# supranational/sppark

Hardware: NVIDIA H100
Metric: BLS12-381 G1 MSM/s @2^26 points (higher is better)
Workload: dtype u32x12 (384-bit Montgomery integers)

## Files before the change

### include/sppark_b200.h

```cpp
#ifndef SPPARK_B200_H
#define SPPARK_B200_H

#include <stddef.h>
#include <stdint.h>

#ifdef __cplusplus
extern "C" {
#endif

typedef struct RustError {
    int   code;
    char *message;
#ifdef __cplusplus
    typedef struct RustError by_value;
#endif
} RustError;


enum { SPPARK_NTT_NN = 0, SPPARK_NTT_NR = 1, SPPARK_NTT_RN = 2, SPPARK_NTT_RR = 3,
       SPPARK_NTT_BB = 4 };
enum { SPPARK_NTT_FORWARD = 0, SPPARK_NTT_INVERSE = 1 };
enum { SPPARK_NTT_STANDARD = 0, SPPARK_NTT_COSET = 1 };


// ... 44 lines not shown
                                     uint32_t lg_blowup, void *stream);

RustError sppark_b200_ntt_batch_dev(int field, void *d_inout, uint32_t lg_domain_size, size_t batch,
                                    int ntt_order, int ntt_direction, int ntt_type, void *stream);
RustError sppark_b200_lde_batch_dev(int field, void *d_out, void *d_in, uint32_t lg_domain_size,
                                    uint32_t lg_blowup, size_t batch, void *stream);
RustError sppark_b200_ntt_batch(int field, size_t device_id, void *inout, uint32_t lg_domain_size,
                                size_t batch, int ntt_order, int ntt_direction, int ntt_type);

RustError sppark_b200_prefix_op_dev(int field, int op, void *d_out, const void *d_inp, size_t len, void *stream);
RustError sppark_b200_div_by_x_minus_z_dev(int field, void *d_inout, size_t len, const void *z, int rotate,
                                           void *stream);
RustError sppark_b200_evaluate_dev(int field, void *d_ret, const void *d_x, size_t n, const void *d_coeffs,
                                   size_t len, void *stream);
RustError sppark_b200_batch_inverse_dev(int field, void *d_out, const void *d_inp, size_t len, void *stream);

RustError sppark_b200_ntt_slab_pass(int field, int which, const void *d_in, void *d_out,
                                    uint32_t lg_domain_size, uint32_t lg_g, uint32_t rank,
                                    int ntt_direction, void *stream);

RustError sppark_b200_ntt_slab_pass_p2p(int field, const void *d_in, void *const *peer_recv,
                                        uint32_t lg_domain_size, uint32_t lg_g, uint32_t rank,
                                        int ntt_direction, void *stream);
RustError sppark_b200_ntt_sharded(int field, void *inout, uint32_t lg_domain_size, int ntt_direction,
                                  const int *device_ids, size_t ndev);

RustError sppark_b200_peer_alloc(size_t bytes, void **d_ptr, void *ipc_handle_64);
RustError sppark_b200_peer_open(const void *ipc_handle_64, void **d_ptr);
RustError sppark_b200_peer_close(void *d_ptr);
RustError sppark_b200_peer_free(void *d_ptr);

RustError sppark_b200_msm(int curve, void *out_jacobian, const void *points_affine,
                          size_t npoints, const void *scalars, size_t ffi_affine_sz);
RustError sppark_b200_msm_ex(int curve, void *out_jacobian, const void *points_affine,
                             size_t npoints, const void *scalars, size_t ffi_affine_sz,
                             int scalars_mont);
RustError sppark_b200_msm_sharded(int curve, void *out_jacobian, const void *points_affine, size_t npoints,
                                  const void *scalars, size_t ffi_affine_sz, int scalars_mont,
                                  const int *device_ids, size_t ndev);
typedef struct sppark_b200_msm_ctx sppark_b200_msm_ctx;
RustError sppark_b200_msm_ctx_create(int curve, const void *points_affine, size_t npoints,
                                     size_t ffi_affine_sz, sppark_b200_msm_ctx **out);
RustError sppark_b200_msm_ctx_invoke(sppark_b200_msm_ctx *ctx, void *out_jacobian, const void *scalars,
                                     size_t npoints, int scalars_mont);
void      sppark_b200_msm_ctx_free(sppark_b200_msm_ctx *ctx);
RustError sppark_b200_msm_dev(int curve, void *out_jacobian, const void *d_points,
                              size_t npoints, const void *d_scalars, void *stream);

RustError sppark_b200_generate_points_dev(int curve, void *d_out, size_t n, void *stream);
RustError sppark_b200_msm_combine(int curve, void *out_jacobian, const void *partials, size_t count);

RustError sppark_b200_selftest_field(int field, int op, size_t n, void *r, const void *a, const void *b);
RustError sppark_b200_selftest_word_field(int field, int op, size_t n, void *r, const void *a, const void *b);

size_t      sppark_b200_ngpus(void);
int         sppark_b200_sm_count(int device_id);
const char *sppark_b200_version(void);
uint64_t    sppark_b200_launch_count(void);
void        sppark_b200_profile_enable(int on);
int         sppark_b200_profile_read(const char **names, float *ms, int cap);

#ifdef __cplusplus
}
#endif
#endif
```

### sppark_b200/_lib.py

```python
import ctypes as C
import os

HERE = os.path.dirname(os.path.abspath(__file__))
LIB_PATH = os.environ.get("SPPARK_B200_LIB") or os.path.join(HERE, "libsppark_b200.so")


class RustError(C.Structure):
    _fields_ = [("code", C.c_int), ("message", C.c_void_p)]


class GpuPtr(C.Structure):
    _fields_ = [("inner", C.c_void_p)]


class SpparkError(RuntimeError):
    def __init__(self, code, message):
        super().__init__(f"sppark_b200 error {code}: {message}")
        self.code = code


_lib = None

_SIGS = {
    "mult_pippenger": [C.c_void_p, C.c_void_p, C.c_size_t, C.c_void_p],
    "mult_pippenger_inf": [C.c_void_p, C.c_void_p, C.c_size_t, C.c_void_p, C.c_size_t],
    "mult_pippenger_fp2_inf": [C.c_void_p, C.c_void_p, C.c_size_t, C.c_void_p, C.c_size_t],
    "compute_ntt": [C.c_size_t, C.c_void_p, C.c_uint32, C.c_int, C.c_int, C.c_int],
    "sppark_b200_ntt": [C.c_int, C.c_size_t, C.c_void_p, C.c_uint32, C.c_int, C.c_int, C.c_int],
    "sppark_b200_ntt_dev": [C.c_int, C.c_void_p, C.c_uint32, C.c_int, C.c_int, C.c_int, C.c_void_p],
    "sppark_b200_lde": [C.c_int, C.c_size_t, C.c_void_p, C.c_uint32, C.c_uint32, C.c_void_p],
    "sppark_b200_ntt_slab_pass": [C.c_int, C.c_int, C.c_void_p, C.c_void_p, C.c_uint32, C.c_uint32, C.c_uint32,
                                  C.c_int, C.c_void_p],
    "sppark_b200_ntt_slab_pass_p2p": [C.c_int, C.c_void_p, C.c_void_p, C.c_uint32, C.c_uint32, C.c_uint32,
                                      C.c_int, C.c_void_p],
    "sppark_b200_peer_alloc": [C.c_size_t, C.POINTER(C.c_void_p), C.c_void_p],
    "sppark_b200_peer_open": [C.c_void_p, C.POINTER(C.c_void_p)],
    "sppark_b200_peer_close": [C.c_void_p],
    "sppark_b200_peer_free": [C.c_void_p],
    "sppark_b200_msm": [C.c_int, C.c_void_p, C.c_void_p, C.c_size_t, C.c_void_p, C.c_size_t],
    "sppark_b200_msm_ex": [C.c_int, C.c_void_p, C.c_void_p, C.c_size_t, C.c_void_p, C.c_size_t, C.c_int],
    "sppark_b200_msm_ctx_create": [C.c_int, C.c_void_p, C.c_size_t, C.c_size_t, C.POINTER(C.c_void_p)],
    "sppark_b200_msm_ctx_invoke": [C.c_void_p, C.c_void_p, C.c_void_p, C.c_size_t, C.c_int],
    "sppark_b200_msm_dev": [C.c_int, C.c_void_p, C.c_void_p, C.c_size_t, C.c_void_p, C.c_void_p],
    "sppark_b200_generate_points_dev": [C.c_int, C.c_void_p, C.c_size_t, C.c_void_p],
    "sppark_b200_msm_combine": [C.c_int, C.c_void_p, C.c_void_p, C.c_size_t],
    "sppark_b200_selftest_field": [C.c_int, C.c_int, C.c_size_t, C.c_void_p, C.c_void_p, C.c_void_p],
    "sppark_b200_lde_powers_dev": [C.c_int, C.c_void_p, C.c_uint32, C.c_void_p],
    "sppark_b200_lde_expand_dev": [C.c_int, C.c_void_p, C.c_void_p, C.c_uint32, C.c_uint32, C.c_void_p],
    "sppark_b200_ntt_batch_dev": [C.c_int, C.c_void_p, C.c_uint32, C.c_size_t, C.c_int, C.c_int, C.c_int, C.c_void_p],
    "sppark_b200_lde_batch_dev": [C.c_int, C.c_void_p, C.c_void_p, C.c_uint32, C.c_uint32, C.c_size_t, C.c_void_p],
    "sppark_b200_ntt_batch": [C.c_int, C.c_size_t, C.c_void_p, C.c_uint32, C.c_size_t, C.c_int, C.c_int, C.c_int],
    "sppark_b200_msm_sharded": [C.c_int, C.c_void_p, C.c_void_p, C.c_size_t, C.c_void_p, C.c_size_t, C.c_int, C.c_void_p, C.c_size_t],
    "sppark_b200_ntt_sharded": [C.c_int, C.c_void_p, C.c_uint32, C.c_int, C.c_void_p, C.c_size_t],
    "sppark_b200_selftest_word_field": [C.c_int, C.c_int, C.c_size_t, C.c_void_p, C.c_void_p, C.c_void_p],
    "sppark_b200_prefix_op_dev": [C.c_int, C.c_int, C.c_void_p, C.c_void_p, C.c_size_t, C.c_void_p],
    "sppark_b200_div_by_x_minus_z_dev": [C.c_int, C.c_void_p, C.c_size_t, C.c_void_p, C.c_int, C.c_void_p],
    "sppark_b200_evaluate_dev": [C.c_int, C.c_void_p, C.c_void_p, C.c_size_t, C.c_void_p, C.c_size_t, C.c_void_p],
    "sppark_b200_batch_inverse_dev": [C.c_int, C.c_void_p, C.c_void_p, C.c_size_t, C.c_void_p],
}

EXPORTS = list(_SIGS) + ["cuda_available", "drop_error_message", "sppark_b200_sm_count", "sppark_b200_ngpus",
                         "sppark_b200_version", "sppark_b200_launch_count",
                         "sppark_b200_profile_enable", "sppark_b200_profile_read",
                         "drop_gpu_ptr_t", "clone_gpu_ptr_t", "sppark_b200_msm_ctx_free", "sppark_b200_gpu_ptr_alloc",
                         "sppark_b200_gpu_ptr_get", "sppark_b200_gpu_ptr_refs"]


def lib():
    global _lib
    if _lib is None:
        if not os.path.exists(LIB_PATH):
            raise ImportError(f"{LIB_PATH} not built: run `python -m sppark_b200.build` "
                              "(there is no CPU fallback)")
        l = C.CDLL(LIB_PATH)
        for name, args in _SIGS.items():
            fn = getattr(l, name)
            fn.argtypes = args
            fn.restype = RustError
        l.cuda_available.restype = C.c_int
        l.drop_error_message.argtypes = [C.c_void_p]
        l.sppark_b200_sm_count.argtypes = [C.c_int]
        l.sppark_b200_version.restype = C.c_char_p
        l.sppark_b200_launch_count.restype = C.c_uint64
        l.sppark_b200_msm_ctx_free.argtypes = [C.c_void_p]
        l.sppark_b200_msm_ctx_free.restype = None
        l.drop_gpu_ptr_t.argtypes = [C.POINTER(GpuPtr)]
        l.clone_gpu_ptr_t.argtypes = [C.POINTER(GpuPtr)]
        l.clone_gpu_ptr_t.restype = GpuPtr
        l.sppark_b200_gpu_ptr_alloc.argtypes = [C.c_size_t]
        l.sppark_b200_gpu_ptr_alloc.restype = GpuPtr
        l.sppark_b200_gpu_ptr_get.argtypes = [C.POINTER(GpuPtr)]
        l.sppark_b200_gpu_ptr_get.restype = C.c_void_p
        l.sppark_b200_gpu_ptr_refs.argtypes = [C.POINTER(GpuPtr)]
        l.sppark_b200_gpu_ptr_refs.restype = C.c_size_t
        l.sppark_b200_profile_enable.argtypes = [C.c_int]
        l.sppark_b200_profile_read.argtypes = [C.POINTER(C.c_char_p), C.POINTER(C.c_float), C.c_int]
        l.sppark_b200_profile_read.restype = C.c_int
        _lib = l
    return _lib


def check(err):
    if err.code != 0:
        msg = C.cast(err.message, C.c_char_p).value.decode() if err.message else ""
        if err.message:
            lib().drop_error_message(err.message)
        raise SpparkError(err.code, msg)
# ... 16 lines not shown
```

### sppark_b200/csrc/msm/msm.cuh

```cuda
#pragma once
#include "../util/gpu.cuh"
#include "msm_core.cuh"
#include "msm_pair.cuh"

namespace msm {

#ifndef SPPARK_B200_ACC_THREADS
# define SPPARK_B200_ACC_THREADS 128
#endif
#ifndef SPPARK_B200_ACC_MIN_BLOCKS
# define SPPARK_B200_ACC_MIN_BLOCKS 3
#endif
constexpr uint32_t ACC_THREADS = SPPARK_B200_ACC_THREADS;
constexpr uint32_t HEAVY_THREADS = 128;

static __global__ void count_kernel(const Config cfg, const uint32_t* scalars, uint32_t* counts)
{
    for (uint32_t i = blockIdx.x * blockDim.x + threadIdx.x; i < cfg.npoints; i += gridDim.x * blockDim.x)
        count_body(cfg, scalars, counts, i);
}


static __global__ void __launch_bounds__(1024)
scan_kernel(const Config cfg, const uint32_t* counts, uint32_t* offsets, uint32_t* cursor,
            uint32_t* ctrl, uint32_t* heavy_list, uint32_t* chunk_map)
{
    __shared__ uint32_t warp_tot[32];
    const uint32_t w = blockIdx.x, nb = 1u << cfg.lg_nb;
    const uint32_t lane = threadIdx.x & 31, wid = threadIdx.x >> 5;
    const size_t base = (size_t)w << cfg.lg_nb;
    uint32_t carry = 0;
    for (uint32_t t0 = 0; t0 < nb; t0 += 4096) {
        const uint32_t b = t0 + threadIdx.x * 4;
        uint4 c = make_uint4(0, 0, 0, 0);
        if (b < nb) c = *reinterpret_cast<const uint4*>(counts + base + b);
        const uint32_t s = c.x + c.y + c.z + c.w;
        uint32_t x = s;
#pragma unroll
        for (uint32_t d = 1; d < 32; d <<= 1) {
            uint32_t y = __shfl_up_sync(0xffffffffu, x, d);
            if (lane >= d) x += y;
        }
        if (lane == 31) warp_tot[wid] = x;
        __syncthreads();
        if (wid == 0) {
            uint32_t t = warp_tot[lane];
#pragma unroll
            for (uint32_t d = 1; d < 32; d <<= 1) {
                uint32_t y = __shfl_up_sync(0xffffffffu, t, d);
                if (lane >= d) t += y;
            }
            warp_tot[lane] = t;
        }
        __syncthreads();
        uint4 r;
        r.x = carry + (wid ? warp_tot[wid - 1] : 0) + x - s;
        r.y = r.x + c.x;
        r.z = r.y + c.y;
        r.w = r.z + c.z;
        carry += warp_tot[31];
        if (b < nb) {
            *reinterpret_cast<uint4*>(offsets + base + b) = r;
            *reinterpret_cast<uint4*>(cursor + base + b) = r;
            const uint32_t cc[4] = {c.x, c.y, c.z, c.w};
#pragma unroll
            for (uint32_t k = 0; k < 4; k++) {
                if (cc[k] > cfg.heavy) {
                    uint32_t h = atomicAdd(&ctrl[1], 1), nch = (cc[k] + cfg.heavy_chunk - 1) / cfg.heavy_chunk;
                    uint32_t first_chunk = atomicAdd(&ctrl[2], nch);
                    heavy_list[3 * h] = (uint32_t)(base + b + k);
                    heavy_list[3 * h + 1] = first_chunk;
                    heavy_list[3 * h + 2] = nch;
                    for (uint32_t q = 0; q < nch; q++) chunk_map[first_chunk + q] = h;
                }
            }
        }
        __syncthreads();
    }
}

static __global__ void scatter_kernel(const Config cfg, const uint32_t* scalars, uint32_t* cursor, uint32_t* sorted,
                                      uint32_t w0, uint32_t w1)
{
    for (uint32_t i = blockIdx.x * blockDim.x + threadIdx.x; i < cfg.npoints; i += gridDim.x * blockDim.x)
        scatter_body(cfg, scalars, cursor, sorted, i, w0, w1);
}

static __global__ void pair_counts_kernel(const Config cfg, const uint32_t* counts, uint32_t* counts1, uint32_t nslots)
{
    for (uint32_t t = blockIdx.x * blockDim.x + threadIdx.x; t < nslots; t += gridDim.x * blockDim.x)
        pair_counts_body(cfg, counts, counts1, t);
}

static __global__ void __launch_bounds__(1024)
pair_scan_kernel(const Config cfg, const uint32_t* counts1, uint32_t* off1, uint32_t* wintotal)
{
    __shared__ uint32_t warp_tot[32];
    const uint32_t w = blockIdx.x, nb = 1u << cfg.lg_nb, lane = threadIdx.x & 31, wid = threadIdx.x >> 5;
    const size_t base = (size_t)w << cfg.lg_nb;
    uint32_t carry = 0;
    for (uint32_t t0 = 0; t0 < nb; t0 += 4096) {
        const uint32_t b = t0 + threadIdx.x * 4;
        uint4 c = make_uint4(0, 0, 0, 0);
        if (b < nb) c = *reinterpret_cast<const uint4*>(counts1 + base + b);
        const uint32_t s = c.x + c.y + c.z + c.w;
        uint32_t x = s;
#pragma unroll
        for (uint32_t d = 1; d < 32; d <<= 1) {
            uint32_t y = __shfl_up_sync(0xffffffffu, x, d);
            if (lane >= d) x += y;
        }
        if (lane == 31) warp_tot[wid] = x;
        __syncthreads();
        if (wid == 0) {
            uint32_t t = warp_tot[lane];
#pragma unroll
            for (uint32_t d = 1; d < 32; d <<= 1) {
                uint32_t y = __shfl_up_sync(0xffffffffu, t, d);
                if (lane >= d) t += y;
            }
            warp_tot[lane] = t;
        }
        __syncthreads();
        uint4 r;
        r.x = carry + (wid ? warp_tot[wid - 1] : 0) + x - s;
        r.y = r.x + c.x;
        r.z = r.y + c.y;
        r.w = r.z + c.z;
        carry += warp_tot[31];
        if (b < nb) *reinterpret_cast<uint4*>(off1 + base + b) = r;
        __syncthreads();
    }
    if (threadIdx.x == 0) wintotal[w] = carry;
}

static __global__ void pair_winbase_kernel(const Config cfg, const uint32_t* wintotal, uint32_t* winbase)
{
    if (blockIdx.x || threadIdx.x) return;
// ... 260 lines not shown
    }
}

template<class F>
__global__ void __launch_bounds__(32)
finish_par_kernel(const Config cfg, const uint32_t* winR, uint32_t* out_jacobian)
{
    __shared__ F slots[Par4<F>::NS];
    if (threadIdx.x >= 4) return;
    Par4<F> p(slots, slots + 4, threadIdx.x);
    {
        const ec::xyzz_t<F> top = load_bucket<F>(winR, cfg.nwins - 1);
        if (p.lane == 0) { slots[Par4<F>::sX] = top.X; slots[Par4<F>::sY] = top.Y; slots[Par4<F>::sZZZ] = top.ZZZ; slots[Par4<F>::sZZ] = top.ZZ; }
        p.sync();
    }
    for (uint32_t w = cfg.nwins - 1; w-- > 0;) {
        for (uint32_t d = 0; d < cfg.wbits; d++) p.dbl();
        p.add(load_bucket<F>(winR, w));
    }
    const bool inf = p.is_inf();
    const F ZZ = slots[Par4<F>::sZZ];
    const F Yf = slots[Par4<F>::sY], ZZZf = slots[Par4<F>::sZZZ];
    const F r = F::mul_shared(p.pick(slots[Par4<F>::sX], Yf, Yf, Yf), p.pick(ZZ, ZZZf, ZZZf, ZZZf));
    if (p.lane < 2)
        for (int k = 0; k < F::N; k++) out_jacobian[p.lane * F::N + k] = inf ? 0 : r.l[k];
    if (p.lane == 2)
        for (int k = 0; k < F::N; k++) out_jacobian[2 * F::N + k] = inf ? 0 : ZZ.l[k];
}

static __global__ void pack_points_kernel(const uint8_t* in, size_t stride, uint32_t words, bool has_flag,
                                   uint32_t* out, uint32_t npoints)
{
    for (uint32_t i = blockIdx.x * blockDim.x + threadIdx.x; i < npoints; i += gridDim.x * blockDim.x) {
        const uint32_t* src = reinterpret_cast<const uint32_t*>(in + (size_t)i * stride);
        bool inf = has_flag && (in[(size_t)i * stride + 4 * words] & 1);
        for (uint32_t k = 0; k < words; k++) out[(size_t)i * words + k] = inf ? 0 : src[k];
    }
}

template<class F>
class msm_t {
    const gpu_t& gpu;
    static constexpr uint32_t PW = 2 * F::N, BW = 4 * F::N, JW = 3 * F::N;

public:
    explicit msm_t(const gpu_t& g) : gpu(g) {}

    struct Job {
        Config cfg;
        size_t nslots, slice_cap;
        uint32_t lg_l, items1;
        uint8_t* blob;
        uint32_t *counts, *offsets, *cursor, *ctrl, *heavy_list, *chunk_map, *partials, *sorted, *buckets;
        uint32_t *R[2], *S[2];
        uint32_t slices_done;
        bool pair;
        size_t pair_bound;
        uint32_t pair_threads;
        uint32_t *counts1, *off1, *wintotal, *winbase, *sums, *pre, *totals;
        cudaStream_t owner;
        Job() : blob(nullptr), owner(nullptr) {}
        Job(const Job&) = delete;
        Job& operator=(const Job&) = delete;
        Job(Job&& o) noexcept { memcpy((void*)this, (const void*)&o, sizeof(Job)); o.blob = nullptr; }
        ~Job() { if (blob) (void)cudaFreeAsync(blob, owner); }
    };

    Job begin(size_t total_points, size_t slice_cap, cudaStream_t stream)
    {
        if (total_points >= (1ull << 31))
            throw cuda_error(-(int)cudaErrorInvalidValue, "msm: npoints must be < 2^31");
        Job j;
        j.cfg = make_config(total_points);
        j.cfg.npoints = (uint32_t)slice_cap;
        j.slice_cap = slice_cap;
        j.nslots = (size_t)j.cfg.nwins << j.cfg.lg_nb;
        j.lg_l = j.cfg.lg_nb > 12 ? j.cfg.lg_nb - 12 : 0;
        j.items1 = j.cfg.nwins << (j.cfg.lg_nb - j.lg_l);
        j.slices_done = 0;
        const size_t entries = (size_t)j.cfg.nwins * slice_cap;
        const size_t heavy_cap = entries / (j.cfg.heavy + 1) + 1;
        const size_t chunk_cap = entries / j.cfg.heavy_chunk + heavy_cap;
        size_t off = 0;
        auto take = [&](size_t bytes) { size_t o = off; off += (bytes + 255) & ~(size_t)255; return o; };
        const size_t o_counts = take(j.nslots * 4), o_offsets = take(j.nslots * 4), o_cursor = take(j.nslots * 4);
        const size_t o_ctrl = take(16), o_heavy = take(heavy_cap * 12), o_cmap = take(chunk_cap * 4);
        const size_t o_partials = take(chunk_cap * BW * 4);
        const size_t o_sorted = take(entries * 4);
        const size_t o_buckets = take(j.nslots * BW * 4);
        const size_t o_r0 = take((size_t)j.items1 * BW * 4), o_s0 = take((size_t)j.items1 * BW * 4);
        const size_t o_r1 = take((size_t)j.items1 * BW * 4 / 2 + 4096), o_s1 = take((size_t)j.items1 * BW * 4 / 2 + 4096);
        const char* pair_env = getenv("SPPARK_B200_MSM_PAIR");
        j.pair = pair_env && atoi(pair_env) != 0 && entries + j.nslots < (1ull << 31);
        j.pair_bound = (entries + std::min<size_t>(entries, j.nslots) + 1) / 2;
        j.pair_threads = (uint32_t)std::min<size_t>((j.pair_bound + PAIR_K - 1) / PAIR_K, (size_t)1 << 21);
        size_t o_c1 = 0, o_o1 = 0, o_wt = 0, o_wb = 0, o_sums = 0, o_pre = 0, o_tot = 0;
        if (j.pair) {
            o_c1 = take(j.nslots * 4); o_o1 = take(j.nslots * 4);
            o_wt = take((j.cfg.nwins + 1) * 4); o_wb = take((j.cfg.nwins + 1) * 4);
            o_sums = take(j.pair_bound * 2 * F::N * 4);
            o_pre = take((size_t)j.pair_threads * PAIR_K * F::N * 4);
            o_tot = take((size_t)j.pair_threads * F::N * 4);
        }
        CUDA_OK(cudaMallocAsync((void**)&j.blob, off, stream));
        j.owner = stream;
        auto U32 = [&](size_t o) { return reinterpret_cast<uint32_t*>(j.blob + o); };
        j.counts = U32(o_counts); j.offsets = U32(o_offsets); j.cursor = U32(o_cursor);
        j.ctrl = U32(o_ctrl); j.heavy_list = U32(o_heavy); j.chunk_map = U32(o_cmap);
        j.partials = U32(o_partials); j.sorted = U32(o_sorted); j.buckets = U32(o_buckets);
        j.R[0] = U32(o_r0); j.S[0] = U32(o_s0); j.R[1] = U32(o_r1); j.S[1] = U32(o_s1);
        j.counts1 = U32(o_c1); j.off1 = U32(o_o1); j.wintotal = U32(o_wt); j.winbase = U32(o_wb);
        j.sums = U32(o_sums); j.pre = U32(o_pre); j.totals = U32(o_tot);
        g_profile.reset();
        return j;
    }

    void slice(Job& j, const uint32_t* d_points, const uint32_t* d_scalars, size_t n, cudaStream_t stream)
    {
        if (n == 0) return;
        Config cfg = j.cfg;
        cfg.npoints = (uint32_t)n;
        cfg.merge = j.slices_done ? 1 : 0;
        const uint32_t sms = (uint32_t)gpu.sm_count();
        g_profile.mark("sort", stream);
        CUDA_OK(cudaMemsetAsync(j.counts, 0, j.nslots * 4, stream));
        CUDA_OK(cudaMemsetAsync(j.ctrl, 0, 16, stream));
        const uint32_t nblk = (uint32_t)std::min<size_t>((n + 255) / 256, (size_t)sms * 16);
        count_kernel<<<nblk, 256, 0, stream>>>(cfg, d_scalars, j.counts);
        COUNT_LAUNCH();
        scan_kernel<<<cfg.nwins, 1024, 0, stream>>>(cfg, j.counts, j.offsets, j.cursor, j.ctrl, j.heavy_list, j.chunk_map);
        COUNT_LAUNCH();
        bool per_window = n >= (1u << 18);
        if (const char* env = getenv("SPPARK_B200_MSM_SCATTER")) per_window = atoi(env) != 0;
        if (per_window) {
            for (uint32_t w = 0; w < cfg.nwins; w++) {
                scatter_kernel<<<nblk, 256, 0, stream>>>(cfg, d_scalars, j.cursor, j.sorted, w, w + 1);
                COUNT_LAUNCH();
            }
        } else {
            scatter_kernel<<<nblk, 256, 0, stream>>>(cfg, d_scalars, j.cursor, j.sorted, 0, cfg.nwins);
            COUNT_LAUNCH();
        }
        CUDA_OK(cudaGetLastError());

        g_profile.mark("accumulate", stream);
        int occ = 1;
        CUDA_OK(cudaOccupancyMaxActiveBlocksPerMultiprocessor(&occ, accumulate_kernel<F>, ACC_THREADS, 0));
        if (occ < 1) occ = 1;
        size_t want = (j.nslots + ACC_THREADS - 1) / ACC_THREADS;
        uint32_t acc_blocks = (uint32_t)std::min<size_t>(want, (size_t)sms * occ);
        if (j.pair) {
            const uint32_t nslots = (uint32_t)j.nslots;
            pair_counts_kernel<<<sms * 8, 256, 0, stream>>>(cfg, j.counts, j.counts1, nslots);
            pair_scan_kernel<<<cfg.nwins, 1024, 0, stream>>>(cfg, j.counts1, j.off1, j.wintotal);
            pair_winbase_kernel<<<1, 32, 0, stream>>>(cfg, j.wintotal, j.winbase);
            const size_t bound = ((size_t)cfg.nwins * n + std::min<size_t>((size_t)cfg.nwins * n, j.nslots) + 1) / 2;
            const size_t per_launch = (size_t)j.pair_threads * PAIR_K;
            for (size_t o0 = 0; o0 < bound; o0 += per_launch) {
                const uint32_t nth = (uint32_t)std::min<size_t>(j.pair_threads, (bound - o0 + PAIR_K - 1) / PAIR_K);
                pair_forward_kernel<F><<<(nth + 127) / 128, 128, 0, stream>>>(
                    cfg, d_points, j.sorted, j.offsets, j.counts, j.counts1, j.off1, j.winbase, (uint32_t)o0, nth, j.pre, j.totals);
                pair_invert_kernel<F><<<((nth + PAIR_M - 1) / PAIR_M + 127) / 128, 128, 0, stream>>>(j.totals, nth);
                pair_backward_kernel<F><<<(nth + 127) / 128, 128, 0, stream>>>(
                    cfg, d_points, j.sorted, j.offsets, j.counts, j.counts1, j.off1, j.winbase, (uint32_t)o0, nth, j.pre, j.totals, j.sums);
                COUNT_LAUNCH(); COUNT_LAUNCH(); COUNT_LAUNCH();
            }
            CUDA_OK(cudaGetLastError());
            g_profile.mark("accumulate_sums", stream);
            accumulate_direct_kernel<F><<<acc_blocks, ACC_THREADS, 0, stream>>>(cfg, j.sums, j.offsets, j.counts, j.buckets,
                                                                               j.ctrl, j.counts1, j.off1, j.winbase);
        } else {
            accumulate_kernel<F><<<acc_blocks, ACC_THREADS, 0, stream>>>(cfg, d_points, j.sorted, j.offsets, j.counts,
                                                                        j.buckets, j.ctrl);
        }
        COUNT_LAUNCH();
        g_profile.mark("heavy", stream);
        heavy_chunks_kernel<F><<<sms * 4, HEAVY_THREADS, HEAVY_THREADS * BW * 4, stream>>>(
            cfg, d_points, j.sorted, j.offsets, j.counts, j.ctrl, j.heavy_list, j.chunk_map, j.partials);
        COUNT_LAUNCH();
        heavy_fold_kernel<F><<<sms, HEAVY_THREADS, HEAVY_THREADS * BW * 4, stream>>>(cfg, j.ctrl, j.heavy_list,
                                                                                    j.partials, j.buckets);
        COUNT_LAUNCH();
        CUDA_OK(cudaGetLastError());
        if (getenv("SPPARK_B200_MSM_DEBUG")) {
            uint32_t dbg[3];
            CUDA_OK(cudaMemcpyAsync(dbg, j.ctrl, 12, cudaMemcpyDeviceToHost, stream));
            CUDA_OK(cudaStreamSynchronize(stream));
            fprintf(stderr, "[msm] slice %u n=%u wbits=%u nwins=%u heavy_thr=%u tasks_claimed=%u nheavy=%u nchunks=%u acc_blocks=%u\n",
                    j.slices_done, cfg.npoints, cfg.wbits, cfg.nwins, cfg.heavy, dbg[0], dbg[1], dbg[2], acc_blocks);
        }
        j.slices_done++;
    }

    void finish(Job& j, uint32_t* d_out, cudaStream_t stream)
    {
        if (j.slices_done == 0) {
// ... 44 lines not shown
```

### sppark_b200/csrc/msm/msm_bls12_381.cu

```cuda
#include "msm_host.cuh"

RustError msm_host_bls12_381(void* out, const void* points, size_t npoints, const void* scalars,
                             size_t stride, bool has_flag, bool mont)
{
    return msm_host<ff::bls12_381_fp_t>(out, points, npoints, scalars, stride, has_flag,
                                        mont ? scalars_from_mont<ff::bls12_381_fr_t> : nullptr);
}
RustError msm_dev_bls12_381(void* out, const void* d_points, size_t npoints, const void* d_scalars, void* stream)
{   return msm_dev<ff::bls12_381_fp_t>(out, d_points, npoints, d_scalars, stream);   }

RustError gen_points_bls12_381(void* d_out, size_t n, void* stream)
{   return gen_points_dev<ff::bls12_381_g1_gen>(d_out, n, stream);   }
RustError combine_bls12_381(void* out, const void* partials, size_t count)
{   return combine_host<ff::bls12_381_fp_t>(out, partials, count);   }

extern "C" RustError mult_pippenger(void* out, const void* points, size_t npoints, const void* scalars)
{   return msm_host_bls12_381(out, points, npoints, scalars, 96, false, false);   }

extern "C" RustError mult_pippenger_inf(void* out, const void* points, size_t npoints,
                                        const void* scalars, size_t ffi_affine_sz)
{   return msm_host_bls12_381(out, points, npoints, scalars, ffi_affine_sz, true, false);   }

template<class F>
__global__ void selftest_kernel(int op, size_t n, uint32_t* r, const uint32_t* a, const uint32_t* b)
// ... 7 lines not shown
    case 1: z = x + y; break;
    case 2: z = x - y; break;
    case 3: z = x.sqr(); break;
    case 4: z = F::mul_shared(x, y); break;
    case 5: z = F::sqr_shared(x); break;
    default: z = F::msub_shared(x, y, y, x.sqr()); break;
    }
    for (int k = 0; k < F::N; k++) r[i * F::N + k] = z.l[k];
}

template<class F>
static RustError selftest(int op, size_t n, void* r, const void* a, const void* b)
{
    try {
        const gpu_t& gpu = select_gpu(-1);
        const stream_t& s = gpu[0];
        size_t bytes = n * F::N * 4;
        dev_ptr_t<uint32_t> da(n * F::N, s), db(n * F::N, s), dr(n * F::N, s);
        s.HtoD(da, a, bytes);
        s.HtoD(db, b, bytes);
        selftest_kernel<F><<<(unsigned)((n + 127) / 128), 128, 0, s>>>(op, n, dr, da, db);
        COUNT_LAUNCH();
        CUDA_OK(cudaGetLastError());
        s.DtoH(r, dr, bytes);
        s.sync();
    } catch (const cuda_error& e) {
        return rust_err(e.code(), e.what());
    }
    return rust_ok();
}

extern "C" RustError sppark_b200_selftest_field(int field, int op, size_t n, void* r, const void* a, const void* b)
{
    switch (field) {
    case 0: return selftest<ff::bls12_381_fp_t>(op, n, r, a, b);
    case 1: return selftest<ff::bls12_381_fr_t>(op, n, r, a, b);
    case 2: return selftest<ff::pallas_fp_t>(op, n, r, a, b);
    case 3: return selftest<ff::vesta_fp_t>(op, n, r, a, b);
    case 4: return selftest<ff::bn254_fp_t>(op, n, r, a, b);
    case 5: return selftest<ff::bn254_fr_t>(op, n, r, a, b);
    case 6: return selftest<ff::bls12_377_fp_t>(op, n, r, a, b);
    case 7: return selftest<ff::bls12_377_fr_t>(op, n, r, a, b);
    default: return rust_err(-(int)cudaErrorInvalidValue, "selftest: unknown field");
    }
}

RustError msm_preload_bls12_381(const void* points, size_t npoints, size_t stride, bool has_flag, void** d_points)
{   return msm_preload<ff::bls12_381_fp_t>(points, npoints, stride, has_flag, d_points);   }
RustError msm_resident_bls12_381(void* out, const void* d_points, size_t npoints, const void* scalars, bool mont)
{
    return msm_host<ff::bls12_381_fp_t>(out, nullptr, npoints, scalars, 0, false, mont ? scalars_from_mont<ff::bls12_381_fr_t> : nullptr,
                      (const uint32_t*)d_points);
}
```

### sppark_b200/csrc/msm/msm_core.cuh

```cuda
#pragma once
#include <algorithm>
#include "../ec/xyzz.cuh"

namespace msm {

struct Config {
    uint32_t wbits;
    uint32_t nwins;
    uint32_t lg_nb;
    uint32_t npoints;
    uint32_t heavy;
    uint32_t heavy_chunk;
    uint32_t merge;
};

HD uint32_t atomic_inc(uint32_t* p, uint32_t v = 1)
{
#if defined(__CUDA_ARCH__)
    return atomicAdd(p, v);
#else
    uint32_t old = *p;
    *p += v;
    return old;
#endif
// ... 4 lines not shown
    uint32_t carry;
    HD explicit Digits(const uint32_t* p) : carry(0)
    {
#if defined(__CUDA_ARCH__)
        uint4 a = reinterpret_cast<const uint4*>(p)[0], b = reinterpret_cast<const uint4*>(p)[1];
        s[0] = a.x; s[1] = a.y; s[2] = a.z; s[3] = a.w;
        s[4] = b.x; s[5] = b.y; s[6] = b.z; s[7] = b.w;
#else
        for (int i = 0; i < 8; i++) s[i] = p[i];
#endif
        s[7] &= 0x7fffffffu;
    }
    HD bool next(uint32_t w, uint32_t c, uint32_t& bucket, uint32_t& neg)
    {
        uint32_t off = w * c, i = off >> 5, sh = off & 31;
        uint32_t lo = i < 8 ? s[i] : 0, hi = i + 1 < 8 ? s[i + 1] : 0;
        uint32_t raw = sh ? (lo >> sh) | (hi << (32 - sh)) : lo;
        raw = (c < 32 ? raw & ((1u << c) - 1) : raw) + carry;
        const uint32_t half = 1u << (c - 1);
        if (raw > half) {
            neg = 1;
            carry = 1;
            raw = (1u << c) - raw;
        } else {
            neg = 0;
            carry = 0;
        }
        bucket = raw - 1;
        return raw != 0;
    }
};

HD void count_body(const Config& cfg, const uint32_t* scalars, uint32_t* counts, uint32_t i)
{
    Digits d(scalars + 8 * (size_t)i);
    for (uint32_t w = 0; w < cfg.nwins; w++) {
        uint32_t b, neg;
        if (d.next(w, cfg.wbits, b, neg))
            atomic_inc(&counts[((size_t)w << cfg.lg_nb) + b]);
    }
}

HD void scatter_body(const Config& cfg, const uint32_t* scalars, uint32_t* cursor,
                     uint32_t* sorted, uint32_t i, uint32_t w0, uint32_t w1)
{
    Digits d(scalars + 8 * (size_t)i);
    for (uint32_t w = 0; w < w1; w++) {
        uint32_t b, neg;
        if (d.next(w, cfg.wbits, b, neg) && w >= w0) {
            uint32_t pos = atomic_inc(&cursor[((size_t)w << cfg.lg_nb) + b]);
            sorted[(size_t)w * cfg.npoints + pos] = i | (neg << 31);
        }
    }
}

template<class F>
HD ec::affine_t<F> load_point(const uint32_t* points, uint32_t entry)
{
    constexpr int W = 2 * F::N;
    const uint32_t* p = points + (size_t)(entry & 0x7fffffffu) * W;
    ec::affine_t<F> a;
#if defined(__CUDA_ARCH__)
    static_assert(W % 4 == 0, "affine point must be a whole number of 16-byte words");
    uint32_t buf[W];
#pragma unroll
    for (int k = 0; k < W / 4; k++) {
        uint4 v = __ldg(reinterpret_cast<const uint4*>(p) + k);
        buf[4 * k] = v.x; buf[4 * k + 1] = v.y; buf[4 * k + 2] = v.z; buf[4 * k + 3] = v.w;
    }
#pragma unroll
    for (int k = 0; k < F::N; k++) { a.X.l[k] = buf[k]; a.Y.l[k] = buf[F::N + k]; }
#else
    for (int k = 0; k < F::N; k++) { a.X.l[k] = p[k]; a.Y.l[k] = p[F::N + k]; }
#endif
    if (entry >> 31) a.Y = a.Y.neg();
    return a;
}

template<class F>
HD void store_bucket(uint32_t* buckets, size_t slot, const ec::xyzz_t<F>& b)
{
    constexpr int W = 4 * F::N;
    uint32_t* p = buckets + slot * W;
#pragma unroll
    for (int k = 0; k < F::N; k++) {
        p[k] = b.X.l[k]; p[F::N + k] = b.Y.l[k]; p[2 * F::N + k] = b.ZZZ.l[k]; p[3 * F::N + k] = b.ZZ.l[k];
    }
}

template<class F>
HD ec::xyzz_t<F> load_bucket(const uint32_t* buckets, size_t slot)
{
    constexpr int W = 4 * F::N;
    const uint32_t* p = buckets + slot * W;
    ec::xyzz_t<F> b;
#pragma unroll
    for (int k = 0; k < F::N; k++) {
        b.X.l[k] = p[k]; b.Y.l[k] = p[F::N + k]; b.ZZZ.l[k] = p[2 * F::N + k]; b.ZZ.l[k] = p[3 * F::N + k];
    }
    return b;
}

template<class F, bool DIRECT = false>
HD void accumulate_body(const Config& cfg, const uint32_t* points, const uint32_t* sorted,
                        const uint32_t* offsets, const uint32_t* counts, uint32_t* buckets,
                        uint32_t* task_counter, const uint32_t* counts1 = nullptr,
// ... 133 lines not shown
```

Measured before the change: 1.901.

## Replace count/scan/scatter bucket sort with two-level binned partition and shared-memory sort

Replaces the global count, scan and per-window scatter passes of the MSM bucket sort with a two-level radix scheme. A shared-memory histogram over coarse bins, a per-window scan, a warp-aggregated partition into a staging buffer, then a per-bin shared-memory counting sort produce counts, offsets and sorted indices. Bins too large for shared memory go through a global-atomic fallback. The aim is to cut scattered global atomics and writes during sorting, at the cost of an extra 8-byte-per-entry staging buffer and more kernel launches. A selftest entry point for the sort is also added.

```diff
diff --git a/include/sppark_b200.h b/include/sppark_b200.h
--- a/include/sppark_b200.h
+++ b/include/sppark_b200.h
@@ -120,6 +120,8 @@
 
 RustError sppark_b200_selftest_field(int field, int op, size_t n, void *r, const void *a, const void *b);
 RustError sppark_b200_selftest_word_field(int field, int op, size_t n, void *r, const void *a, const void *b);
+RustError sppark_b200_selftest_msm_sort(size_t n, uint32_t wbits, uint32_t cap, const void *scalars, void *counts,
+                                        void *offsets, void *sorted, void *heavy_slots, uint32_t *info);
 
 size_t      sppark_b200_ngpus(void);
 int         sppark_b200_sm_count(int device_id);
diff --git a/sppark_b200/_lib.py b/sppark_b200/_lib.py
--- a/sppark_b200/_lib.py
+++ b/sppark_b200/_lib.py
@@ -53,6 +53,8 @@
     "sppark_b200_msm_sharded": [C.c_int, C.c_void_p, C.c_void_p, C.c_size_t, C.c_void_p, C.c_size_t, C.c_int, C.c_void_p, C.c_size_t],
     "sppark_b200_ntt_sharded": [C.c_int, C.c_void_p, C.c_uint32, C.c_int, C.c_void_p, C.c_size_t],
     "sppark_b200_selftest_word_field": [C.c_int, C.c_int, C.c_size_t, C.c_void_p, C.c_void_p, C.c_void_p],
+    "sppark_b200_selftest_msm_sort": [C.c_size_t, C.c_uint32, C.c_uint32, C.c_void_p, C.c_void_p, C.c_void_p,
+                                      C.c_void_p, C.c_void_p, C.c_void_p],
     "sppark_b200_prefix_op_dev": [C.c_int, C.c_int, C.c_void_p, C.c_void_p, C.c_size_t, C.c_void_p],
     "sppark_b200_div_by_x_minus_z_dev": [C.c_int, C.c_void_p, C.c_size_t, C.c_void_p, C.c_int, C.c_void_p],
     "sppark_b200_evaluate_dev": [C.c_int, C.c_void_p, C.c_void_p, C.c_size_t, C.c_void_p, C.c_size_t, C.c_void_p],
diff --git a/sppark_b200/csrc/msm/msm.cuh b/sppark_b200/csrc/msm/msm.cuh
--- a/sppark_b200/csrc/msm/msm.cuh
+++ b/sppark_b200/csrc/msm/msm.cuh
@@ -14,76 +14,232 @@
 constexpr uint32_t ACC_THREADS = SPPARK_B200_ACC_THREADS;
 constexpr uint32_t HEAVY_THREADS = 128;
 
-static __global__ void count_kernel(const Config cfg, const uint32_t* scalars, uint32_t* counts)
-{
-    for (uint32_t i = blockIdx.x * blockDim.x + threadIdx.x; i < cfg.npoints; i += gridDim.x * blockDim.x)
-        count_body(cfg, scalars, counts, i);
-}
-
-
-static __global__ void __launch_bounds__(1024)
-scan_kernel(const Config cfg, const uint32_t* counts, uint32_t* offsets, uint32_t* cursor,
-            uint32_t* ctrl, uint32_t* heavy_list, uint32_t* chunk_map)
+constexpr uint32_t HIST_THREADS = 1024;
+constexpr uint32_t HIST_SMEM_WORDS = 56 * 1024;
+constexpr uint32_t SORT_THREADS = 512;
+constexpr uint32_t SORT_CAP = 24576;
+
+template<class Load, class Visit>
+__device__ uint32_t block_exclusive_scan(uint32_t len, Load load, Visit visit)
 {
     __shared__ uint32_t warp_tot[32];
-    const uint32_t w = blockIdx.x, nb = 1u << cfg.lg_nb;
-    const uint32_t lane = threadIdx.x & 31, wid = threadIdx.x >> 5;
-    const size_t base = (size_t)w << cfg.lg_nb;
+    const uint32_t lane = threadIdx.x & 31, wid = threadIdx.x >> 5, nw = blockDim.x >> 5;
     uint32_t carry = 0;
-    for (uint32_t t0 = 0; t0 < nb; t0 += 4096) {
-        const uint32_t b = t0 + threadIdx.x * 4;
-        uint4 c = make_uint4(0, 0, 0, 0);
-        if (b < nb) c = *reinterpret_cast<const uint4*>(counts + base + b);
-        const uint32_t s = c.x + c.y + c.z + c.w;
+    for (uint32_t t0 = 0; t0 < len; t0 += 4 * blockDim.x) {
+        const uint32_t b = t0 + 4 * threadIdx.x;
+        uint32_t c[4];
+#pragma unroll
+        for (uint32_t k = 0; k < 4; k++) c[k] = b + k < len ? load(b + k) : 0;
+        const uint32_t s = c[0] + c[1] + c[2] + c[3];
         uint32_t x = s;
 #pragma unroll
         for (uint32_t d = 1; d < 32; d <<= 1) {
-            uint32_t y = __shfl_up_sync(0xffffffffu, x, d);
+            const uint32_t y = __shfl_up_sync(0xffffffffu, x, d);
             if (lane >= d) x += y;
         }
         if (lane == 31) warp_tot[wid] = x;
         __syncthreads();
         if (wid == 0) {
-            uint32_t t = warp_tot[lane];
+            uint32_t t = lane < nw ? warp_tot[lane] : 0;
 #pragma unroll
             for (uint32_t d = 1; d < 32; d <<= 1) {
-                uint32_t y = __shfl_up_sync(0xffffffffu, t, d);
+                const uint32_t y = __shfl_up_sync(0xffffffffu, t, d);
                 if (lane >= d) t += y;
             }
             warp_tot[lane] = t;
         }
         __syncthreads();
-        uint4 r;
-        r.x = carry + (wid ? warp_tot[wid - 1] : 0) + x - s;
-        r.y = r.x + c.x;
-        r.z = r.y + c.y;
-        r.w = r.z + c.z;
+        uint32_t r = carry + (wid ? warp_tot[wid - 1] : 0) + x - s;
         carry += warp_tot[31];
-        if (b < nb) {
-            *reinterpret_cast<uint4*>(offsets + base + b) = r;
-            *reinterpret_cast<uint4*>(cursor + base + b) = r;
-            const uint32_t cc[4] = {c.x, c.y, c.z, c.w};
 #pragma unroll
-            for (uint32_t k = 0; k < 4; k++) {
-                if (cc[k] > cfg.heavy) {
-                    uint32_t h = atomicAdd(&ctrl[1], 1), nch = (cc[k] + cfg.heavy_chunk - 1) / cfg.heavy_chunk;
-                    uint32_t first_chunk = atomicAdd(&ctrl[2], nch);
-                    heavy_list[3 * h] = (uint32_t)(base + b + k);
-                    heavy_list[3 * h + 1] = first_chunk;
-                    heavy_list[3 * h + 2] = nch;
-                    for (uint32_t q = 0; q < nch; q++) chunk_map[first_chunk + q] = h;
-                }
+        for (uint32_t k = 0; k < 4; k++) {
+            if (b + k < len) visit(b + k, c[k], r);
+            r += c[k];
+        }
+        __syncthreads();
+    }
+    return carry;
+}
+
+static __global__ void __launch_bounds__(HIST_THREADS)
+bin_hist_kernel(const Config cfg, uint32_t lg_bins, const uint32_t* scalars, uint32_t wpg, uint32_t* bin_count)
+{
+    extern __shared__ uint32_t hist[];
+    const uint32_t w0 = blockIdx.y * wpg, w1 = min(w0 + wpg, cfg.nwins), nctr = (w1 - w0) << lg_bins;
+    const uint32_t lane = threadIdx.x & 31;
+    for (uint32_t k = threadIdx.x; k < nctr; k += blockDim.x) hist[k] = 0;
+    __syncthreads();
+    for (uint32_t i0 = blockIdx.x * blockDim.x + (threadIdx.x & ~31u); i0 < cfg.npoints; i0 += gridDim.x * blockDim.x) {
+        const uint32_t i = i0 + lane;
+        for_each_digit(cfg, lg_bins, scalars, i, i < cfg.npoints, w1,
+                       [&](uint32_t w, bool nz, uint32_t bin, uint32_t, uint32_t) {
+            if (w < w0) return;
+            const uint32_t key = nz ? bin - (w0 << lg_bins) : ~0u;
+            const uint32_t peers = __match_any_sync(0xffffffffu, key);
+            if (nz && lane == __ffs(peers) - 1) atomicAdd(&hist[key], __popc(peers));
+        });
+    }
+    __syncthreads();
+    for (uint32_t k = threadIdx.x; k < nctr; k += blockDim.x)
+        if (hist[k]) atomicAdd(&bin_count[((size_t)w0 << lg_bins) + k], hist[k]);
+}
+
+static __global__ void __launch_bounds__(1024)
+bin_scan_kernel(uint32_t lg_bins, const uint32_t* bin_count, uint32_t* bin_base, uint32_t* bin_cur)
+{
+    const size_t row = (size_t)blockIdx.x << lg_bins;
+    block_exclusive_scan(1u << lg_bins, [&](uint32_t j) { return bin_count[row + j]; },
+                         [&](uint32_t j, uint32_t, uint32_t off) { bin_base[row + j] = off; bin_cur[row + j] = off; });
+}
+
+static __global__ void __launch_bounds__(256)
+partition_kernel(const Config cfg, uint32_t lg_bins, const uint32_t* scalars, uint32_t* bin_cur, uint2* staging)
+{
+    const uint32_t lane = threadIdx.x & 31;
+    for (uint32_t i0 = blockIdx.x * blockDim.x + (threadIdx.x & ~31u); i0 < cfg.npoints; i0 += gridDim.x * blockDim.x) {
+        const uint32_t i = i0 + lane;
+        for_each_digit(cfg, lg_bins, scalars, i, i < cfg.npoints, cfg.nwins,
+                       [&](uint32_t w, bool nz, uint32_t bin, uint32_t b, uint32_t entry) {
+            const uint32_t peers = __match_any_sync(0xffffffffu, nz ? bin : ~0u);
+            const uint32_t leader = __ffs(peers) - 1;
+            uint32_t pos = 0;
+            if (nz && lane == leader) pos = atomicAdd(&bin_cur[bin], __popc(peers));
+            pos = __shfl_sync(0xffffffffu, pos, leader) + __popc(peers & ((1u << lane) - 1));
+            if (nz) staging[(size_t)w * cfg.npoints + pos] = make_uint2(entry, b);
+        });
+    }
+}
+
+static __global__ void __launch_bounds__(SORT_THREADS)
+bin_sort_kernel(const Config cfg, uint32_t lg_bins, uint32_t cap, const uint2* staging, const uint32_t* bin_count,
+                const uint32_t* bin_base, uint32_t* counts, uint32_t* offsets, uint32_t* sorted, uint32_t* ctrl,
+                uint32_t* heavy_list, uint32_t* chunk_map, uint32_t* overflow)
+{
+    extern __shared__ uint32_t sm[];
+    const uint32_t w = blockIdx.x >> lg_bins, bin = blockIdx.x & ((1u << lg_bins) - 1);
+    uint32_t b0, nbk;
+    if (!bin_buckets(cfg, lg_bins, w, bin, b0, nbk)) return;
+    const uint32_t cnt = bin_count[blockIdx.x], base = bin_base[blockIdx.x];
+    const size_t t0 = ((size_t)w << cfg.lg_nb) + b0;
+    if (last_bin(cfg, lg_bins, w, bin))
+        for (uint32_t b = b0 + nbk + threadIdx.x; b < (1u << cfg.lg_nb); b += blockDim.x)
+            offsets[((size_t)w << cfg.lg_nb) + b] = base + cnt;
+    if (cnt > cap) {
+        if (threadIdx.x == 0) overflow[atomicAdd(&ctrl[3], 1)] = blockIdx.x;
+        return;
+    }
+    uint32_t *run = sm, *cur = sm + cap;
+    for (uint32_t k = threadIdx.x; k < nbk; k += blockDim.x) cur[k] = 0;
+    __syncthreads();
+    const uint2* src = staging + (size_t)w * cfg.npoints + base;
+    for (uint32_t k = threadIdx.x; k < cnt; k += blockDim.x) atomicAdd(&cur[src[k].y - b0], 1);
+    __syncthreads();
+    block_exclusive_scan(nbk, [&](uint32_t j) { return cur[j]; }, [&](uint32_t j, uint32_t c, uint32_t off) {
+        counts[t0 + j] = c;
+        offsets[t0 + j] = base + off;
+        cur[j] = off;
+        register_heavy(cfg, (uint32_t)(t0 + j), c, ctrl, heavy_list, chunk_map);
+    });
+    for (uint32_t k = threadIdx.x; k < cnt; k += blockDim.x) {
+        const uint2 e = src[k];
+        run[atomicAdd(&cur[e.y - b0], 1)] = e.x;
+    }
+    __syncthreads();
+    uint32_t* dst = sorted + (size_t)w * cfg.npoints + base;
+    for (uint32_t k = threadIdx.x; k < cnt; k += blockDim.x) dst[k] = run[k];
+}
+
+template<bool PLACE>
+__global__ void __launch_bounds__(256)
+overflow_kernel(const Config cfg, uint32_t lg_bins, const uint2* staging, const uint32_t* bin_count,
+                const uint32_t* bin_base, const uint32_t* ctrl, const uint32_t* overflow, uint32_t* slots,
+                uint32_t* sorted)
+{
+    const uint32_t lane = threadIdx.x & 31, nov = ctrl[3];
+    for (uint32_t o = 0; o < nov; o++) {
+        const uint32_t g = overflow[o], w = g >> lg_bins, cnt = bin_count[g];
+        const uint2* src = staging + (size_t)w * cfg.npoints + bin_base[g];
+        uint32_t* row = slots + ((size_t)w << cfg.lg_nb);
+        for (uint32_t k0 = blockIdx.x * blockDim.x + (threadIdx.x & ~31u); k0 < cnt; k0 += gridDim.x * blockDim.x) {
+            const uint32_t k = k0 + lane;
+            const uint2 e = k < cnt ? src[k] : make_uint2(0, ~0u);
+            const uint32_t peers = __match_any_sync(0xffffffffu, e.y);
+            const uint32_t leader = __ffs(peers) - 1;
+            uint32_t pos = 0;
+            if (k < cnt && lane == leader) pos = atomicAdd(&row[e.y], __popc(peers));
+            if (PLACE) {
+                pos = __shfl_sync(0xffffffffu, pos, leader) + __popc(peers & ((1u << lane) - 1));
+                if (k < cnt) sorted[(size_t)w * cfg.npoints + pos] = e.x;
             }
         }
-        __syncthreads();
-    }
-}
-
-static __global__ void scatter_kernel(const Config cfg, const uint32_t* scalars, uint32_t* cursor, uint32_t* sorted,
-                                      uint32_t w0, uint32_t w1)
-{
-    for (uint32_t i = blockIdx.x * blockDim.x + threadIdx.x; i < cfg.npoints; i += gridDim.x * blockDim.x)
-        scatter_body(cfg, scalars, cursor, sorted, i, w0, w1);
+    }
+}
+
+static __global__ void __launch_bounds__(1024)
+overflow_scan_kernel(const Config cfg, uint32_t lg_bins, const uint32_t* bin_base, const uint32_t* overflow,
+                     const uint32_t* counts, uint32_t* offsets, uint32_t* cursor, uint32_t* ctrl,
+                     uint32_t* heavy_list, uint32_t* chunk_map)
+{
+    const uint32_t nov = ctrl[3];
+    for (uint32_t o = blockIdx.x; o < nov; o += gridDim.x) {
+        const uint32_t g = overflow[o], w = g >> lg_bins, base = bin_base[g];
+        uint32_t b0, nbk;
+        bin_buckets(cfg, lg_bins, w, g & ((1u << lg_bins) - 1), b0, nbk);
+        const size_t t0 = ((size_t)w << cfg.lg_nb) + b0;
+        block_exclusive_scan(nbk, [&](uint32_t j) { return counts[t0 + j]; }, [&](uint32_t j, uint32_t c, uint32_t off) {
+            offsets[t0 + j] = base + off;
+            cursor[t0 + j] = base + off;
+            register_heavy(cfg, (uint32_t)(t0 + j), c, ctrl, heavy_list, chunk_map);
+        });
+    }
+}
+
+struct SortBufs {
+    uint32_t *counts, *offsets, *cursor, *ctrl, *heavy_list, *chunk_map, *sorted;
+    uint32_t *bin_count, *bin_base, *bin_cur, *overflow;
+    uint2* staging;
+};
+
+inline bool sort_profile() { const char* e = getenv("SPPARK_B200_MSM_SORT_PROFILE"); return e && atoi(e) != 0; }
+
+inline void sort_slice(const Config& cfg, uint32_t cap, const uint32_t* d_scalars, const SortBufs& s, uint32_t sms,
+                       cudaStream_t stream)
+{
+    const uint32_t lg_bins = sort_lg_bins(cfg, cfg.npoints);
+    const size_t nbins = (size_t)cfg.nwins << lg_bins, nslots = (size_t)cfg.nwins << cfg.lg_nb;
+    const bool marks = sort_profile();
+    CUDA_OK(cudaFuncSetAttribute(bin_hist_kernel, cudaFuncAttributeMaxDynamicSharedMemorySize, HIST_SMEM_WORDS * 4));
+    CUDA_OK(cudaFuncSetAttribute(bin_sort_kernel, cudaFuncAttributeMaxDynamicSharedMemorySize,
+                                 (SORT_CAP + (1u << SORT_SMAX)) * 4));
+    CUDA_OK(cudaMemsetAsync(s.counts, 0, nslots * 4, stream));
+    CUDA_OK(cudaMemsetAsync(s.ctrl, 0, 16, stream));
+    CUDA_OK(cudaMemsetAsync(s.bin_count, 0, nbins * 4, stream));
+    const uint32_t wpg = std::min(cfg.nwins, HIST_SMEM_WORDS >> lg_bins);
+    const uint32_t ngroups = (cfg.nwins + wpg - 1) / wpg;
+    const uint32_t hist_blk = (uint32_t)std::min<size_t>((cfg.npoints + HIST_THREADS - 1) / HIST_THREADS, sms);
+    bin_hist_kernel<<<dim3(hist_blk, ngroups), HIST_THREADS, ((size_t)wpg << lg_bins) * 4, stream>>>(
+        cfg, lg_bins, d_scalars, wpg, s.bin_count);
+    COUNT_LAUNCH();
+    bin_scan_kernel<<<cfg.nwins, 1024, 0, stream>>>(lg_bins, s.bin_count, s.bin_base, s.bin_cur);
+    COUNT_LAUNCH();
+    if (marks) g_profile.mark("sort_partition", stream);
+    const uint32_t part_blk = (uint32_t)std::min<size_t>((cfg.npoints + 255) / 256, (size_t)sms * 8);
+    partition_kernel<<<part_blk, 256, 0, stream>>>(cfg, lg_bins, d_scalars, s.bin_cur, s.staging);
+    COUNT_LAUNCH();
+    if (marks) g_profile.mark("sort_bins", stream);
+    bin_sort_kernel<<<(uint32_t)nbins, SORT_THREADS, (cap + (1u << SORT_SMAX)) * 4, stream>>>(
+        cfg, lg_bins, cap, s.staging, s.bin_count, s.bin_base, s.counts, s.offsets, s.sorted, s.ctrl,
+        s.heavy_list, s.chunk_map, s.overflow);
+    COUNT_LAUNCH();
+    if (marks) g_profile.mark("sort_overflow", stream);
+    overflow_kernel<false><<<sms * 4, 256, 0, stream>>>(cfg, lg_bins, s.staging, s.bin_count, s.bin_base, s.ctrl,
+                                                        s.overflow, s.counts, s.sorted);
+    overflow_scan_kernel<<<sms, 1024, 0, stream>>>(cfg, lg_bins, s.bin_base, s.overflow, s.counts, s.offsets, s.cursor,
+                                                   s.ctrl, s.heavy_list, s.chunk_map);
+    overflow_kernel<true><<<sms * 4, 256, 0, stream>>>(cfg, lg_bins, s.staging, s.bin_count, s.bin_base, s.ctrl,
+                                                       s.overflow, s.cursor, s.sorted);
+    COUNT_LAUNCH(); COUNT_LAUNCH(); COUNT_LAUNCH();
+    CUDA_OK(cudaGetLastError());
 }
 
 static __global__ void pair_counts_kernel(const Config cfg, const uint32_t* counts, uint32_t* counts1, uint32_t nslots)
@@ -450,6 +606,8 @@
         uint32_t lg_l, items1;
         uint8_t* blob;
         uint32_t *counts, *offsets, *cursor, *ctrl, *heavy_list, *chunk_map, *partials, *sorted, *buckets;
+        uint32_t *bin_count, *bin_base, *bin_cur, *overflow;
+        uint2* staging;
         uint32_t *R[2], *S[2];
         uint32_t slices_done;
         bool pair;
@@ -482,6 +640,9 @@
         size_t off = 0;
         auto take = [&](size_t bytes) { size_t o = off; off += (bytes + 255) & ~(size_t)255; return o; };
         const size_t o_counts = take(j.nslots * 4), o_offsets = take(j.nslots * 4), o_cursor = take(j.nslots * 4);
+        const size_t nbins = (size_t)j.cfg.nwins << sort_lg_bins(j.cfg, slice_cap);
+        const size_t o_bcount = take(nbins * 4), o_bbase = take(nbins * 4), o_bcur = take(nbins * 4), o_over = take(nbins * 4);
+        const size_t o_staging = take(entries * 8);
         const size_t o_ctrl = take(16), o_heavy = take(heavy_cap * 12), o_cmap = take(chunk_cap * 4);
         const size_t o_partials = take(chunk_cap * BW * 4);
         const size_t o_sorted = take(entries * 4);
@@ -506,6 +667,8 @@
         j.counts = U32(o_counts); j.offsets = U32(o_offsets); j.cursor = U32(o_cursor);
         j.ctrl = U32(o_ctrl); j.heavy_list = U32(o_heavy); j.chunk_map = U32(o_cmap);
         j.partials = U32(o_partials); j.sorted = U32(o_sorted); j.buckets = U32(o_buckets);
+        j.bin_count = U32(o_bcount); j.bin_base = U32(o_bbase); j.bin_cur = U32(o_bcur); j.overflow = U32(o_over);
+        j.staging = reinterpret_cast<uint2*>(j.blob + o_staging);
         j.R[0] = U32(o_r0); j.S[0] = U32(o_s0); j.R[1] = U32(o_r1); j.S[1] = U32(o_s1);
         j.counts1 = U32(o_c1); j.off1 = U32(o_o1); j.wintotal = U32(o_wt); j.winbase = U32(o_wb);
         j.sums = U32(o_sums); j.pre = U32(o_pre); j.totals = U32(o_tot);
@@ -521,25 +684,9 @@
         cfg.merge = j.slices_done ? 1 : 0;
         const uint32_t sms = (uint32_t)gpu.sm_count();
         g_profile.mark("sort", stream);
-        CUDA_OK(cudaMemsetAsync(j.counts, 0, j.nslots * 4, stream));
-        CUDA_OK(cudaMemsetAsync(j.ctrl, 0, 16, stream));
-        const uint32_t nblk = (uint32_t)std::min<size_t>((n + 255) / 256, (size_t)sms * 16);
-        count_kernel<<<nblk, 256, 0, stream>>>(cfg, d_scalars, j.counts);
-        COUNT_LAUNCH();
-        scan_kernel<<<cfg.nwins, 1024, 0, stream>>>(cfg, j.counts, j.offsets, j.cursor, j.ctrl, j.heavy_list, j.chunk_map);
-        COUNT_LAUNCH();
-        bool per_window = n >= (1u << 18);
-        if (const char* env = getenv("SPPARK_B200_MSM_SCATTER")) per_window = atoi(env) != 0;
-        if (per_window) {
-            for (uint32_t w = 0; w < cfg.nwins; w++) {
-                scatter_kernel<<<nblk, 256, 0, stream>>>(cfg, d_scalars, j.cursor, j.sorted, w, w + 1);
-                COUNT_LAUNCH();
-            }
-        } else {
-            scatter_kernel<<<nblk, 256, 0, stream>>>(cfg, d_scalars, j.cursor, j.sorted, 0, cfg.nwins);
-            COUNT_LAUNCH();
-        }
-        CUDA_OK(cudaGetLastError());
+        const SortBufs sb{j.counts, j.offsets, j.cursor, j.ctrl, j.heavy_list, j.chunk_map, j.sorted,
+                          j.bin_count, j.bin_base, j.bin_cur, j.overflow, j.staging};
+        sort_slice(cfg, SORT_CAP, d_scalars, sb, sms, stream);
 
         g_profile.mark("accumulate", stream);
         int occ = 1;
diff --git a/sppark_b200/csrc/msm/msm_bls12_381.cu b/sppark_b200/csrc/msm/msm_bls12_381.cu
--- a/sppark_b200/csrc/msm/msm_bls12_381.cu
+++ b/sppark_b200/csrc/msm/msm_bls12_381.cu
@@ -83,3 +83,45 @@
     return msm_host<ff::bls12_381_fp_t>(out, nullptr, npoints, scalars, 0, false, mont ? scalars_from_mont<ff::bls12_381_fr_t> : nullptr,
                       (const uint32_t*)d_points);
 }
+
+extern "C" RustError sppark_b200_selftest_msm_sort(size_t n, uint32_t wbits, uint32_t cap, const void* scalars,
+                                                   void* counts, void* offsets, void* sorted, void* heavy_slots,
+                                                   uint32_t* info)
+{
+    using namespace msm;
+    if (n == 0 || n >= (1ull << 31) || wbits < 3 || wbits > 24 || cap > SORT_CAP)
+        return rust_err(-(int)cudaErrorInvalidValue, "selftest_msm_sort: bad arguments");
+    try {
+        const gpu_t& gpu = select_gpu(-1);
+        const stream_t& s = gpu[0];
+        Config cfg = make_config(n);
+        cfg.wbits = wbits;
+        cfg.nwins = (256 + wbits - 1) / wbits;
+        cfg.lg_nb = wbits - 1;
+        const size_t nslots = (size_t)cfg.nwins << cfg.lg_nb, entries = (size_t)cfg.nwins * n;
+        const size_t nbins = (size_t)cfg.nwins << sort_lg_bins(cfg, n);
+        const size_t heavy_cap = entries / (cfg.heavy + 1) + 1, chunk_cap = entries / cfg.heavy_chunk + heavy_cap;
+        dev_ptr_t<uint32_t> d_sc(8 * n, s), d_counts(nslots, s), d_offsets(nslots, s), d_cursor(nslots, s);
+        dev_ptr_t<uint32_t> d_ctrl(4, s), d_heavy(3 * heavy_cap, s), d_cmap(chunk_cap, s), d_sorted(entries, s);
+        dev_ptr_t<uint32_t> d_bcount(nbins, s), d_bbase(nbins, s), d_bcur(nbins, s), d_over(nbins, s);
+        dev_ptr_t<uint32_t> d_staging(2 * entries, s);
+        s.HtoD(d_sc, scalars, 32 * n);
+        const SortBufs sb{d_counts, d_offsets, d_cursor, d_ctrl, d_heavy, d_cmap, d_sorted,
+                          d_bcount, d_bbase, d_bcur, d_over, reinterpret_cast<uint2*>((uint32_t*)d_staging)};
+        sort_slice(cfg, cap ? cap : SORT_CAP, d_sc, sb, (uint32_t)gpu.sm_count(), s);
+        uint32_t ctrl[4];
+        s.DtoH(ctrl, d_ctrl, 16);
+        s.DtoH(counts, d_counts, nslots * 4);
+        s.DtoH(offsets, d_offsets, nslots * 4);
+        s.DtoH(sorted, d_sorted, entries * 4);
+        s.sync();
+        std::vector<uint32_t> hl(3 * (size_t)ctrl[1] + 1);
+        if (ctrl[1]) s.DtoH(hl.data(), d_heavy, 12 * (size_t)ctrl[1]);
+        s.sync();
+        for (uint32_t h = 0; h < ctrl[1]; h++) static_cast<uint32_t*>(heavy_slots)[h] = hl[3 * h];
+        info[0] = cfg.nwins; info[1] = cfg.heavy; info[2] = ctrl[1]; info[3] = sort_lg_bins(cfg, n); info[4] = ctrl[3];
+    } catch (const cuda_error& e) {
+        return rust_err(e.code(), e.what());
+    }
+    return rust_ok();
+}
diff --git a/sppark_b200/csrc/msm/msm_core.cuh b/sppark_b200/csrc/msm/msm_core.cuh
--- a/sppark_b200/csrc/msm/msm_core.cuh
+++ b/sppark_b200/csrc/msm/msm_core.cuh
@@ -80,6 +80,65 @@
             sorted[(size_t)w * cfg.npoints + pos] = i | (neg << 31);
         }
     }
+}
+
+constexpr uint32_t SORT_SMAX = 12;
+constexpr uint32_t SORT_LG_FILL = 13;
+
+HD uint32_t top_window_bits(const Config& cfg)
+{
+    const uint32_t e = 255 - (cfg.nwins - 1) * cfg.wbits;
+    return e < cfg.lg_nb ? e : cfg.lg_nb;
+}
+HD uint32_t window_bits(const Config& cfg, uint32_t w) { return w + 1 < cfg.nwins ? cfg.lg_nb : top_window_bits(cfg); }
+HD uint32_t bin_shift(const Config& cfg, uint32_t lg_bins, uint32_t w)
+{
+    const uint32_t ub = window_bits(cfg, w);
+    return ub > lg_bins ? ub - lg_bins : 0;
+}
+
+inline uint32_t sort_lg_bins(const Config& cfg, size_t n)
+{
+    int lg_n = 0;
+    while (((size_t)1 << lg_n) < n) lg_n++;
+    int lb = std::max(std::min(lg_n - (int)SORT_LG_FILL, 15), (int)cfg.lg_nb - (int)SORT_SMAX);
+    lb = std::min(lb, (int)cfg.lg_nb);
+    return (uint32_t)std::max(lb, 2);
+}
+
+HD bool bin_buckets(const Config& cfg, uint32_t lg_bins, uint32_t w, uint32_t bin, uint32_t& b0, uint32_t& nbk)
+{
+    const uint32_t s = bin_shift(cfg, lg_bins, w), ub = window_bits(cfg, w);
+    b0 = bin << s;
+    nbk = 1u << s;
+    return b0 < (1u << ub);
+}
+
+HD bool last_bin(const Config& cfg, uint32_t lg_bins, uint32_t w, uint32_t bin)
+{   return ((bin + 1) << bin_shift(cfg, lg_bins, w)) == (1u << window_bits(cfg, w));   }
+
+template<class Fn>
+HD void for_each_digit(const Config& cfg, uint32_t lg_bins, const uint32_t* scalars, uint32_t i, bool valid,
+                       uint32_t w_end, Fn fn)
+{
+    Digits d(scalars + 8 * (size_t)(valid ? i : 0));
+    for (uint32_t w = 0; w < w_end; w++) {
+        uint32_t b, neg;
+        const bool nz = d.next(w, cfg.wbits, b, neg) && valid;
+        fn(w, nz, (w << lg_bins) + (nz ? b >> bin_shift(cfg, lg_bins, w) : 0), b, i | (neg << 31));
+    }
+}
+
+HD void register_heavy(const Config& cfg, uint32_t t, uint32_t cnt, uint32_t* ctrl, uint32_t* heavy_list,
+                       uint32_t* chunk_map)
+{
+    if (cnt <= cfg.heavy) return;
+    const uint32_t h = atomic_inc(&ctrl[1]), nch = (cnt + cfg.heavy_chunk - 1) / cfg.heavy_chunk;
+    const uint32_t first_chunk = atomic_inc(&ctrl[2], nch);
+    heavy_list[3 * h] = t;
+    heavy_list[3 * h + 1] = first_chunk;
+    heavy_list[3 * h + 2] = nch;
+    for (uint32_t q = 0; q < nch; q++) chunk_map[first_chunk + q] = h;
 }
 
 template<class F>
```

After: 1.972, median of 6. +3.7%, better.
